# Excalibur-SLE/spmv

Measured on AMD Instinct MI355X. Metric: fp64 CG iters/sec (SpMV effective GB/s vs HBM roofline), higher is better.
Workload: dtype f64

## Files before the change

spmv_amd/csrc/hip/common.h:

```cpp
#pragma once

#include <mutex>
#include <vector>

#include <hip/hip_runtime.h>

#include <cstdint>
#include <cstdlib>

#include "spmv_hip.h"

struct spmv_hip_ctx {
  int device = 0;
  int num_cus = 0;
  hipStream_t stream = nullptr;
  int dot_blocks = 0;
  int64_t blas1_nt_min_elems = (int64_t)1 << 24;
  int64_t lx_min_nnz = (int64_t)1 << 20;
  int64_t lx_max_x_bytes = INT64_MAX;
  int lx_dma = 1;
  int lx_codes = 1;
  int lx_narrow_values = 1;
  int release_csr = 0;
  int64_t xw_min_nnz = (int64_t)1 << 20;
  int64_t xw_min_x_bytes = (int64_t)128 << 20;
  int xw_probe = 1;
  int csr_in_place = 0;
  int64_t lat_min_nnz = (int64_t)1 << 20;
  int bake_general = 1;
  int wdia_half = 1;
  int const_diagonals = 1;
  int const_tile = 4;
  int64_t sj_min_nnz = (int64_t)1 << 20;
  int sj_max_chunks = 432;
  int sj_wpb = 0;
  int sj_unit = 0;
  int sj_sigma = 1;
  int sym_sj_long_permille = 50;
  int sym_sj_long_rows = 1;
  int put_timeout_ms = 60000;
  std::vector<const int32_t*> watched;
  std::mutex watched_mutex;
  int poisson_skew_ppm = 0;
  int poisson_stencil = 7;
};

enum PeerWait : int32_t {
  kWaitNone = 0,
  kWaitPutFree = 1,
  kWaitPutData = 2,
  kWaitReduceSlot = 3
};
constexpr int kPeerErrLabels = 12;
constexpr int kPeerErrWords = kPeerErrLabels + 16;

// ... 95 lines not shown
```

spmv_amd/csrc/hip/csr_plan.h:

```cpp
#pragma once

#include "common.h"

#include <chrono>
#include <cstdio>

constexpr int kRows = kBlock;

typedef double f64x2 __attribute__((ext_vector_type(2)));
typedef float f32x4 __attribute__((ext_vector_type(4)));
typedef int i32x2 __attribute__((ext_vector_type(2)));
typedef int i32x4 __attribute__((ext_vector_type(4)));

template <typename T>
struct VecOf;
template <>
struct VecOf<double> {
  static constexpr int V = 2;
  using val_t = f64x2;
  using col_t = i32x2;
};
template <>
struct VecOf<float> {
  static constexpr int V = 4;
// ... 70 lines not shown
  }
}
__device__ __forceinline__ int order_slot_decode(const RowBlockOrder& ord,
                                                 int raw)
{
  const int rb = __builtin_amdgcn_readfirstlane(raw);
  return rb < ord.num_row_blocks ? rb : -1;
}
#endif

constexpr int kLxMaxWin = 16;
constexpr int kLxRec = 36;
constexpr int kLxCap = 1344;
constexpr int kLxGap = 16;
constexpr int kLxwPiece = 128;
constexpr int kLxwMaxPieces = 16;
constexpr int kLxwPieces0 = 4;
constexpr int kLxwNpMask = 0xff;
constexpr int kLxwOwnShift = 8;
constexpr int kLxwOwnMask = 0xfffff;
constexpr int kLxwCodedBit = 30;
constexpr int kLxwDict0 = kLxwPieces0 + kLxwMaxPieces;
constexpr int kLxwDictSize = 16;
constexpr int kLxwRec = 28;
__host__ __device__ constexpr int64_t lx_code_bytes(int64_t nnz)
{
  return (((nnz + 1) >> 1) + 16 + 15) & ~(int64_t)15;
}
__host__ __device__ constexpr int64_t lx32_len(int64_t nnz)
{
  return (nnz + 3) & ~(int64_t)3;
}
constexpr int kLxwAlign = 4;
constexpr int kXwMaxWin = 8;
constexpr int kXwFirst0 = kLxwPieces0 + kLxwMaxPieces;
constexpr int kXwDelta0 = kXwFirst0 + kXwMaxWin;
constexpr int kXwRec = 36;

constexpr int kLatMaxOff = 8;
constexpr int kLatRec = 12;
constexpr int kWdiaMaxOff = 32;

struct PlanTrace {
  bool on;
  std::chrono::steady_clock::time_point t0;
  const char* who;
  explicit PlanTrace(const char* w)
      : on(getenv("SPMV_PLAN_TRACE") != nullptr), t0(std::chrono::steady_clock::now()),
        who(w)
  {
  }
  void mark(const char* what) const
  {
    if (!on)
      return;
    (void)hipDeviceSynchronize();
    fprintf(stderr, "%s %-14s %9.3f ms\n", who, what,
            std::chrono::duration<double, std::milli>(std::chrono::steady_clock::now()
                                                      - t0)
                .count());
  }
};

template <typename T>
static inline bool aligned16(const T* p)
{
// ... 139 lines not shown
  int mv_form = 0;
  int mv_native = 1;
  int32_t* row_list = nullptr;
  int rowlist_exact = 0;
  int32_t num_listed = 0;
  int nt_store = 0;
  int plan_us = 0;
  int plan_mem_us = 0;
  int values_changed_us = 0;
  const int32_t* rowptr0 = nullptr;
  const int32_t* colind0 = nullptr;
  int released = 0;
  int no_new_forms = 0;
  bool structure_baked() const
  {
    return row_list || lx_lidx || lat_tab || slat_mask || t_ptr || lxw_rec
           || xw_rec || wdia_val || sj_lenperm;
  }
  uint16_t* lx_lidx = nullptr;
  int32_t* lx_tab = nullptr;
  int lx = 0;
  int lx_chunks = 2;
  int lx_staged = 0;
  int lx_blocks = 0;
  int32_t* lxw_rec = nullptr;
  int lxw = 0;
  int lxw_max_cnt = 0;
  int lxw_max_pieces = 0;
  int lxw_blocks_per_cu = 0;
  uint8_t* lx_code = nullptr;
  int lx4 = 0;
  int lx4_blocks = 0;
  int lx4_lut = 1;
  float* lx_val32 = nullptr;
  const void* lx32_values0 = nullptr;
  int lx_v32 = 0;
  int32_t* xw_rec = nullptr;
  int xw = 0;
  int xw_staged = 0;
  int xw_max_cnt = 0, xw_max_pieces = 0;
  struct XwProbe* xw_probe = nullptr;
  int32_t* lat_tab = nullptr;
  uint8_t* lat_mask = nullptr;
  int lat = 0;
  int lat_blocks = 0;
  int lat_blocks_per_cu = 4;
  int lat_xcd_group = 0;
  int lat_chain = 1;

  int lattice_d1 = 0, lattice_d2 = 0;

  int32_t* zw_table = nullptr;
  int zw_slots = 0;
  int zw_grid = 0;
  int zw_segments = 0;
  int64_t zw_d2 = 0;
  int zwalk = 0;

  RowBlockOrder row_block_order(int nrb) const
  {
    RowBlockOrder o;
    o.table = nullptr;
    o.num_slots = 0;
    o.xcd_group = xcd_group;
    o.num_row_blocks = nrb;
    o.nt_store = nt_store;
// ... 54 lines not shown
int spmv_zwalk_table_device(const spmv_hip_csr_plan* pl, int64_t rows,
                            int64_t d2, int grid, int segments, bool force,
                            int32_t** table, int* slots, int* segs);
int spmv_walk_grid(const spmv_hip_csr_plan* pl);
int spmv_slat_build(spmv_hip_csr_plan* pl, const int32_t* rowptr,
                    const int32_t* colind);
void spmv_slat_free(spmv_hip_csr_plan* pl);
int spmv_slat_grid(const spmv_hip_csr_plan* pl);
int spmv_slat_run_f64(const spmv_hip_csr_plan* pl, hipStream_t st,
                      const int32_t* rowptr, const double* values,
                      const double* diagonal, double alpha, const double* in,
                      double beta, double* out, DotOut dot);
int spmv_slat_run_f32(const spmv_hip_csr_plan* pl, hipStream_t st,
                      const int32_t* rowptr, const float* values,
                      const float* diagonal, float alpha, const float* in,
                      float beta, float* out);
void spmv_sdia_free(spmv_hip_csr_plan* pl);
int spmv_sdia_tile_build(spmv_hip_csr_plan* pl, int R, int segments, bool force);
int spmv_sdia_bake_f64(spmv_hip_csr_plan* pl, const double* values,
                       const double* diagonal, hipStream_t st);
int spmv_sdia_bake_f32(spmv_hip_csr_plan* pl, const float* values,
                       const float* diagonal, hipStream_t st);
int spmv_sdia_grid(const spmv_hip_csr_plan* pl);
int spmv_sdia_bake_f32f64(spmv_hip_csr_plan* pl, const float* values32,
                          hipStream_t st);
int spmv_sdia_run_f32f64(const spmv_hip_csr_plan* pl, hipStream_t st,
                         double alpha, const double* in, double beta,
                         double* out, DotOut dot);
int spmv_sdia_run_f64(const spmv_hip_csr_plan* pl, hipStream_t st, double alpha,
                      const double* in, double beta, double* out, DotOut dot);
int spmv_sdia_run_f32(const spmv_hip_csr_plan* pl, hipStream_t st, float alpha,
                      const float* in, float beta, float* out);
int spmv_lxw_grid(const spmv_hip_csr_plan* pl, int elem_bytes);
int spmv_lxw_run_f64(const spmv_hip_csr_plan* pl, hipStream_t st,
                     const int32_t* rowptr, const int32_t* colind,
                     const double* values, double alpha, const double* in,
                     double beta, double* out, DotOut dot);
int spmv_lxw_run_f32f64(const spmv_hip_csr_plan* pl, hipStream_t st,
                        const int32_t* rowptr, const int32_t* colind,
                        const float* values, double alpha, const double* in,
                        double beta, double* out, DotOut dot);
int spmv_xw_grid(const spmv_hip_csr_plan* pl, int elem_bytes);
int spmv_xw_run_f64(const spmv_hip_csr_plan* pl, hipStream_t st,
                    const int32_t* rowptr, const int32_t* colind,
                    const double* values, double alpha, const double* in,
                    double beta, double* out, DotOut dot);
int spmv_xw_run_f32(const spmv_hip_csr_plan* pl, hipStream_t st,
                    const int32_t* rowptr, const int32_t* colind,
                    const float* values, float alpha, const float* in,
                    float beta, float* out);
int spmv_lxw_run_f32(const spmv_hip_csr_plan* pl, hipStream_t st,
                     const int32_t* rowptr, const int32_t* colind,
                     const float* values, float alpha, const float* in,
                     float beta, float* out);
void spmv_wdia_free(spmv_hip_csr_plan* pl);
int spmv_wdia_walk_build(spmv_hip_csr_plan* pl, int segments, bool force);
int spmv_wdia_box_build(spmv_hip_csr_plan* pl, int R, int segments, bool force);
int spmv_wdia_hbox_build(spmv_hip_csr_plan* pl, int on);
int spmv_wdia_bake_f64(spmv_hip_csr_plan* pl, const double* values,
                       hipStream_t st);
int spmv_wdia_bake_f32(spmv_hip_csr_plan* pl, const float* values,
                       hipStream_t st);
int spmv_wdia_run_f64(const spmv_hip_csr_plan* pl, hipStream_t st, double alpha,
                      const double* in, double beta, double* out, DotOut dot);
int spmv_wdia_run_f32(const spmv_hip_csr_plan* pl, hipStream_t st, float alpha,
                      const float* in, float beta, float* out);
// ... 46 lines not shown
```

spmv_amd/csrc/hip/runtime.hip:

```cpp
#include "common.h"

#include <cstdio>
#include <cstring>
#include <new>

bool spmv_ctx_watch(spmv_hip_ctx* ctx, const int32_t* word, bool add)
{
  std::lock_guard<std::mutex> lock(ctx->watched_mutex);
  auto& ws = ctx->watched;
  if (add) {
    try {
      ws.push_back(word);
    } catch (...) {
      return false;
    }
    return true;
  }
  for (size_t i = 0; i < ws.size(); ++i)
    if (ws[i] == word) {
      ws[i] = ws.back();
      ws.pop_back();
      break;
    }
  return true;
// ... 111 lines not shown
  SPMV_REQUIRE(ctx && device_id);
  *device_id = ctx->device;
  return SPMV_HIP_OK;
}

int spmv_hip_num_cus(const spmv_hip_ctx* ctx, int* num_cus)
{
  SPMV_REQUIRE(ctx && num_cus);
  *num_cus = ctx->num_cus;
  return SPMV_HIP_OK;
}

int spmv_hip_ctx_get_option(const spmv_hip_ctx* ctx, const char* key, int64_t* value)
{
  SPMV_REQUIRE(ctx && key && value);
  if (!strcmp(key, "release_csr"))
    *value = ctx->release_csr;
  else if (!strcmp(key, "put_timeout_ms"))
    *value = ctx->put_timeout_ms;
  else if (!strcmp(key, "xw_min_nnz"))
    *value = ctx->xw_min_nnz;
  else if (!strcmp(key, "xw_min_x_bytes"))
    *value = ctx->xw_min_x_bytes;
  else if (!strcmp(key, "xw_probe"))
    *value = ctx->xw_probe;
  else if (!strcmp(key, "csr_in_place"))
    *value = ctx->csr_in_place;
  else if (!strcmp(key, "lx_min_nnz"))
    *value = ctx->lx_min_nnz;
  else if (!strcmp(key, "lat_min_nnz"))
    *value = ctx->lat_min_nnz;
  else if (!strcmp(key, "lx_narrow_values"))
    *value = ctx->lx_narrow_values;
  else if (!strcmp(key, "sj_min_nnz"))
    *value = ctx->sj_min_nnz;
  else
    return SPMV_HIP_EINVAL;
  return SPMV_HIP_OK;
}

int spmv_hip_ctx_set_option(spmv_hip_ctx* ctx, const char* key, int64_t value)
{
  SPMV_REQUIRE(ctx && key);
  if (!strcmp(key, "blas1_nt_min_elems")) {
    SPMV_REQUIRE(value >= 0);
    ctx->blas1_nt_min_elems = value;
    return SPMV_HIP_OK;
  }
  if (!strcmp(key, "lx_max_x_bytes")) {
    SPMV_REQUIRE(value >= 0);
    ctx->lx_max_x_bytes = value;
    return SPMV_HIP_OK;
  }
  if (!strcmp(key, "lx_min_nnz")) {
    SPMV_REQUIRE(value >= 0);
    ctx->lx_min_nnz = value;
    return SPMV_HIP_OK;
  }
  if (!strcmp(key, "release_csr")) {
    SPMV_REQUIRE(value == 0 || value == 1);
    ctx->release_csr = (int)value;
    return SPMV_HIP_OK;
  }
  if (!strcmp(key, "xw_min_x_bytes")) {
    SPMV_REQUIRE(value >= 0);
    ctx->xw_min_x_bytes = value;
// ... 7 lines not shown
  if (!strcmp(key, "xw_probe")) {
    SPMV_REQUIRE(value == 0 || value == 1);
    ctx->xw_probe = (int)value;
    return SPMV_HIP_OK;
  }
  if (!strcmp(key, "csr_in_place")) {
    SPMV_REQUIRE(value == 0 || value == 1);
    ctx->csr_in_place = (int)value;
    return SPMV_HIP_OK;
  }
  if (!strcmp(key, "lat_min_nnz")) {
    SPMV_REQUIRE(value >= 0);
    ctx->lat_min_nnz = value;
    return SPMV_HIP_OK;
  }
  if (!strcmp(key, "poisson_skew_ppm")) {
    SPMV_REQUIRE(value >= 0 && value < 1000000);
    ctx->poisson_skew_ppm = (int)value;
    return SPMV_HIP_OK;
  }
  if (!strcmp(key, "lx_dma")) {
    SPMV_REQUIRE(value == 0 || value == 1);
    ctx->lx_dma = (int)value;
    return SPMV_HIP_OK;
  }
  if (!strcmp(key, "lx_codes")) {
    SPMV_REQUIRE(value == 0 || value == 1);
    ctx->lx_codes = (int)value;
    return SPMV_HIP_OK;
  }
  if (!strcmp(key, "lx_narrow_values")) {
    SPMV_REQUIRE(value == 0 || value == 1);
    ctx->lx_narrow_values = (int)value;
    return SPMV_HIP_OK;
  }
  if (!strcmp(key, "poisson_stencil")) {
    SPMV_REQUIRE(value == 7 || value == 27);
    ctx->poisson_stencil = (int)value;
    return SPMV_HIP_OK;
  }
  if (!strcmp(key, "const_diagonals")) {
    SPMV_REQUIRE(value == 0 || value == 1);
    ctx->const_diagonals = (int)value;
    return SPMV_HIP_OK;
  }
  if (!strcmp(key, "const_tile")) {
    SPMV_REQUIRE(value == 1 || value == 2 || value == 4);
    ctx->const_tile = (int)value;
    return SPMV_HIP_OK;
  }
  if (!strcmp(key, "wdia_half")) {
    SPMV_REQUIRE(value == 0 || value == 1);
    ctx->wdia_half = (int)value;
    return SPMV_HIP_OK;
  }
  if (!strcmp(key, "sj_min_nnz")) {
    SPMV_REQUIRE(value >= 0);
    ctx->sj_min_nnz = value;
    return SPMV_HIP_OK;
  }
  if (!strcmp(key, "sj_max_chunks")) {
    SPMV_REQUIRE(value >= 8 && value <= 432);
    ctx->sj_max_chunks = (int)value;
    return SPMV_HIP_OK;
  }
  if (!strcmp(key, "sj_wpb")) {
// ... 254 lines not shown
```

spmv_amd/csrc/hip/spmv_csr_forms.hip:

```cpp
#include "csr_plan.h"

#include <hipcub/hipcub.hpp>

#include <algorithm>
#include <chrono>
#include <cstring>
#include <new>
#include <utility>
#include <vector>

#include "plan_scratch.h"

namespace
{

template <int ITEMS>
__global__ __launch_bounds__(kBlock) void lx_build_kernel(
    int32_t num_rows, int32_t num_cols, const int32_t* __restrict__ rowptr,
    const int32_t* __restrict__ colind, uint16_t* __restrict__ lidx,
    int32_t* __restrict__ tab, int num_row_blocks, int end_bit, int align,
    int pad, int cap, int32_t* __restrict__ wrec, int32_t* __restrict__ stat,
    int xw)
{
  using Sort = hipcub::BlockRadixSort<int32_t, kBlock, ITEMS, int32_t>;
// ... 108 lines not shown
      int np = 0;
      for (int k = 0; k < total_windows; ++k)
        for (int c = s_ws[k]; c < s_we[k]; c += kLxwPiece)
          wr[kLxwPieces0 + np++] = c;
      wr[0] = total_windows;
      int own = -1;
      for (int k = 0; k < total_windows; ++k)
        if (s_ws[k] <= r0 && r0 + nr <= s_we[k])
          own = s_wo[k] + (r0 - s_ws[k]);
      wr[3] = np | ((own + 1) << kLxwOwnShift);
      if (cnt > *(volatile int*)&stat[0])
        atomicMax(&stat[0], cnt);
      if (np > *(volatile int*)&stat[1])
        atomicMax(&stat[1], np);
      if (xw)
        atomicAdd(&stat[2], 1);
    }
  }
}

constexpr int kLx4Dmin = -kRows;
constexpr int kLx4Words = (kLxwMaxPieces * kLxwPiece + kRows + 31) / 32;
__global__ __launch_bounds__(kBlock) void lx4_encode_kernel(
    int32_t num_rows, const int32_t* __restrict__ rowptr,
    const uint16_t* __restrict__ lidx, int32_t* __restrict__ wrec,
    uint32_t* __restrict__ code, int num_row_blocks, int32_t* __restrict__ stat)
{
  constexpr int CAP = kBlock * 16;
  __shared__ uint32_t s_bits[kLx4Words];
  __shared__ int32_t s_rank[kLx4Words + 1];
  __shared__ int32_t s_dict[kLxwDictSize];
  __shared__ uint32_t s_pack[CAP / 8 + 2];
  const int t = threadIdx.x;
  int coded = 0;
  for (int rb = blockIdx.x; rb < num_row_blocks; rb += gridDim.x) {
    int32_t* wr = wrec + (int64_t)rb * kLxwRec;
    const int32_t a = wr[1], cnt = wr[2];
    const int nwin = wr[0];
    __syncthreads();
    if (nwin < 0 || cnt <= 0 || cnt > CAP)
      continue;
    const int32_t a0 = a & ~7;
    const int nwords = (int)(((int64_t)a + cnt + 7 - a0) >> 3);
    for (int w = t; w < kLx4Words; w += kBlock)
      s_bits[w] = 0;
    for (int w = t; w < nwords; w += kBlock)
      s_pack[w] = 0;
    if (t < kLxwDictSize)
      s_dict[t] = 0;
    __syncthreads();
    const int32_t r = rb * kRows + t;
    int32_t lo = 0, hi = 0;
    if (r < num_rows) {
      lo = rowptr[r];
      hi = rowptr[r + 1];
    }
    for (int32_t j = lo; j < hi; ++j) {
      const int b = (int)lidx[j] - t - kLx4Dmin;
      atomicOr(&s_bits[b >> 5], 1u << (b & 31));
    }
    __syncthreads();
    if (t == 0) {
      int n = 0;
      for (int w = 0; w < kLx4Words; ++w) {
        s_rank[w] = n;
        n += __popc(s_bits[w]);
      }
// ... 2 lines not shown
    __syncthreads();
    if (s_rank[kLx4Words] > kLxwDictSize)
      continue;
    for (int w = t; w < kLx4Words; w += kBlock) {
      uint32_t m = s_bits[w];
      int k = s_rank[w];
      while (m) {
        const int b = __ffs(m) - 1;
        m &= m - 1;
        s_dict[k++] = w * 32 + b + kLx4Dmin;
      }
    }
    for (int32_t j = lo; j < hi; ++j) {
      const int b = (int)lidx[j] - t - kLx4Dmin;
      const uint32_t c
          = (uint32_t)(s_rank[b >> 5] + __popc(s_bits[b >> 5] & ((1u << (b & 31)) - 1u)));
      const int q = j - a0;
      atomicOr(&s_pack[q >> 3], c << ((q & 7) * 4));
    }
    __syncthreads();
    for (int w = t; w < nwords; w += kBlock) {
      const bool whole = (w > 0 || a0 == a) && (int64_t)a0 + 8 * (w + 1) <= (int64_t)a + cnt;
      uint32_t* dst = code + ((int64_t)a0 >> 3) + w;
      if (whole)
        *dst = s_pack[w];
      else if (s_pack[w])
        atomicOr(dst, s_pack[w]);
    }
    if (t < kLxwDictSize / 2)
      wr[kLxwDict0 + t] = (s_dict[2 * t] & 0xffff) | (s_dict[2 * t + 1] << 16);
    if (t == 0) {
      wr[3] |= 1 << kLxwCodedBit;
      ++coded;
    }
  }
  if (t == 0 && coded)
    atomicAdd(&stat[0], coded);
}

struct NonEmptyRow {
  const int32_t* rowptr;
  __device__ bool operator()(int i) const { return rowptr[i + 1] > rowptr[i]; }
};

}

void xw_probe_free(spmv_hip_csr_plan* pl)
{
  if (!pl->xw_probe)
    return;
  for (auto& e : pl->xw_probe->ev)
    for (hipEvent_t& h : e)
      if (h) {
        (void)hipEventDestroy(h);
        h = nullptr;
      }
  delete pl->xw_probe;
  pl->xw_probe = nullptr;
}

void xw_probe_drop_events(XwProbe* pb)
{
  for (auto& e : pb->ev)
    for (hipEvent_t& h : e)
      if (h) {
        (void)hipEventDestroy(h);
        h = nullptr;
      }
}

// ... 39 lines not shown
  const size_t cap = (size_t)(pl->nnz < n ? pl->nnz : n);
  PlanScratch<int32_t> d_count;
  PlanScratch<void> tmp;
  SPMV_CHECK_HIP(spmv_plan_malloc(&pl->row_list, sizeof(int32_t) * (cap ? cap : 1)));
  hipError_t e = d_count.alloc(1);
  hipcub::CountingInputIterator<int32_t> first(0);
  NonEmptyRow pred{rowptr};
  if (e == hipSuccess)
    e = plan_cub(tmp, [&](void* t, size_t& tb) {
      return hipcub::DeviceSelect::If(t, tb, first, pl->row_list, d_count.get(), n,
                                      pred, st);
    });
  int32_t count = 0;
  if (e == hipSuccess)
    e = plan_fetch(&count, d_count.get(), 1, st);
  tmp.reset();
  d_count.reset();
  if (e != hipSuccess) {
    plan_drop(pl->row_list);
    return static_cast<int>(e);
  }
  pl->num_listed = count;
  return SPMV_HIP_OK;
}

void spmv_free_lx(spmv_hip_csr_plan* pl)
{
  plan_drop(pl->lx_lidx);
  plan_drop(pl->lx_tab);
  plan_drop(pl->lxw_rec);
  plan_drop(pl->lx_code);
  pl->lx = pl->lx_staged = pl->lx_blocks = 0;
  pl->lxw = pl->lxw_max_cnt = pl->lxw_max_pieces = 0;
  pl->lx4 = pl->lx4_blocks = 0;
  spmv_lx32_free(pl);
}

static int build_lx_codes(spmv_hip_csr_plan* pl, const int32_t* rowptr, int nrb,
                          hipStream_t st)
{
  const size_t bytes = (size_t)lx_code_bytes(pl->nnz);
  PlanScratch<int32_t> d_stat;
  hipError_t e = spmv_plan_malloc(&pl->lx_code, bytes);
  if (e == hipSuccess)
    e = d_stat.alloc(1);
  if (e == hipSuccess)
    e = hipMemsetAsync(pl->lx_code, 0, bytes, st);
  if (e == hipSuccess)
    e = hipMemsetAsync(d_stat.get(), 0, sizeof(int32_t), st);
  int32_t coded = 0;
  if (e == hipSuccess) {
    int grid = pl->ctx->num_cus * 8;
    grid = grid > nrb ? nrb : grid;
    hipLaunchKernelGGL(lx4_encode_kernel, dim3(grid), dim3(kBlock), 0, st,
                       pl->num_rows, rowptr, pl->lx_lidx, pl->lxw_rec,
                       reinterpret_cast<uint32_t*>(pl->lx_code), nrb, d_stat.get());
    e = hipGetLastError();
  }
  if (e == hipSuccess)
    e = plan_fetch(&coded, d_stat.get(), 1, st);
  d_stat.reset();
  if (e != hipSuccess || coded == 0) {
    (void)hipGetLastError();
    plan_drop(pl->lx_code);
    pl->lx4 = pl->lx4_blocks = 0;
    return e == hipSuccess || e == hipErrorOutOfMemory ? SPMV_HIP_OK
                                                       : static_cast<int>(e);
  }
  pl->lx4_blocks = coded;
  pl->lx4 = 1;
  return SPMV_HIP_OK;
}

namespace
{

__device__ __forceinline__ bool lx32_exact(double v)
{
  const double a = fabs(v);
  if (!(a == 0.0 || (a >= 0x1p-126 && a <= 0x1.fffffep+127)))
    return false;
  return __double_as_longlong((double)(float)v) == __double_as_longlong(v);
}

__global__ __launch_bounds__(kBlock) void lx32_check_kernel(
    int64_t nnz, const double* __restrict__ values, int32_t* __restrict__ flag)
{
  const f64x2* v2 = reinterpret_cast<const f64x2*>(values);
  const int64_t pairs = nnz >> 1;
  bool bad = false;
  for (int64_t i = (int64_t)blockIdx.x * kBlock + threadIdx.x; i < pairs;
       i += (int64_t)gridDim.x * kBlock) {
    const f64x2 v = v2[i];
    bad |= !lx32_exact(v.x) || !lx32_exact(v.y);
  }
  if ((nnz & 1) && blockIdx.x == 0 && threadIdx.x == 0)
    bad |= !lx32_exact(values[nnz - 1]);
  if (bad)
    atomicOr(flag, 1);
}

__global__ __launch_bounds__(kBlock) void lx32_convert_kernel(
// ... 496 lines not shown
```

spmv_amd/csrc/hip/spmv_csr_plan.hip:

```cpp
#include "csr_plan.h"

#include <hipcub/hipcub.hpp>

#include <algorithm>
#include <chrono>
#include <cstring>
#include <new>
#include <utility>
#include <vector>

#include "plan_scratch.h"

thread_local int64_t spmv_plan_mem_ns = 0;

namespace
{
struct MemClock {
  spmv_hip_csr_plan* pl;
  int64_t t0;
  explicit MemClock(spmv_hip_csr_plan* p = nullptr) : pl(p), t0(spmv_plan_mem_ns) {}
  ~MemClock()
  {
    if (pl)
      pl->plan_mem_us += (int)((spmv_plan_mem_ns - t0) / 1000);
// ... 55 lines not shown
               : 0;
  if (pl->sdia32_val || pl->wdia32_val || pl->sj_val32)
    return 0;
  if (pl->sdia && pl->sdia_val && pl->sdia_general && pl->sdia_values0)
    return 3;
  if (pl->wdia && pl->wdia_val && pl->wdia_values0)
    return 3;
  if (pl->sj && pl->sj_val && pl->sj_values0 && pl->sj_nlong == 0 && pl->num_cols >= 2)
    return 3;
  return 0;
}

extern "C" {

int spmv_hip_csr_plan_create(spmv_hip_ctx* ctx, int32_t num_rows,
                             int32_t num_cols, int64_t num_non_zeros,
                             const int32_t* rowptr, const int32_t* colind,
                             int symmetric, int algo, spmv_hip_csr_plan** plan)
{
  SPMV_REQUIRE(ctx && plan && num_rows >= 0 && num_cols >= 0
               && num_non_zeros >= 0);
  SPMV_REQUIRE(num_non_zeros == 0 || (rowptr && colind));
  if (num_non_zeros > 0) {
    SPMV_SET_DEVICE(ctx);
    SPMV_CHECK_HIP(hipStreamSynchronize(spmv_stream(ctx, nullptr)));
  }
  const auto t_begin = std::chrono::steady_clock::now();
  if (num_non_zeros > INT32_MAX)
    return SPMV_HIP_ERANGE;
  spmv_hip_csr_plan* pl = new (std::nothrow) spmv_hip_csr_plan;
  if (!pl)
    return SPMV_HIP_ENOMEM;
  pl->ctx = ctx;
  MemClock mem_clock(pl);
  pl->num_rows = num_rows;
  pl->num_cols = num_cols;
  pl->nnz = num_non_zeros;
  pl->symmetric = symmetric != 0;
  pl->rowptr0 = rowptr;
  pl->colind0 = colind;
  const double avg = num_rows > 0 ? (double)num_non_zeros / num_rows : 0.0;
  if (algo == SPMV_HIP_ALGO_AUTO) {
    if (!symmetric && num_non_zeros > 0 && num_non_zeros * 4 < num_rows)
      algo = SPMV_HIP_ALGO_ROWLIST;
    else
      algo = (avg <= 64.0 || num_non_zeros >= ctx->sj_min_nnz)
                 ? SPMV_HIP_ALGO_ROWBLOCK
                 : SPMV_HIP_ALGO_VECTOR;
  }
  if (algo < SPMV_HIP_ALGO_ROWBLOCK || algo > SPMV_HIP_ALGO_ROWLIST
      || (algo == SPMV_HIP_ALGO_ROWLIST && (symmetric || num_non_zeros == 0))) {
    mem_clock.pl = nullptr;
    delete pl;
    return SPMV_HIP_EINVAL;
  }
  pl->algo = algo;
  if (algo == SPMV_HIP_ALGO_ROWLIST) {
    int rc = spmv_build_row_list(pl, rowptr);
    if (rc != SPMV_HIP_OK) {
      mem_clock.pl = nullptr;
      delete pl;
      return rc;
    }
  }
  int lpr = 4;
  while (lpr < 64 && lpr < avg / 2)
// ... 343 lines not shown
  } else if (!strcmp(key, "xcd_group")) {
    SPMV_REQUIRE(value >= 0 && value <= 4096);
    plan->xcd_group = value;
  } else if (!strcmp(key, "sym_window")) {
    SPMV_REQUIRE(value >= 0 && value <= 4096 && value % 256 == 0);
    plan->sym_window = value;
  } else if (!strcmp(key, "sym_rows")) {
    SPMV_REQUIRE(value == 512 || value == 1024 || value == 2048);
    plan->sym_rows = value;
  } else if (!strcmp(key, "blocks_per_cu")) {
    SPMV_REQUIRE(value >= 1 && value <= kBlocksPerCU);
    plan->blocks_per_cu = value;
    if (plan->zw_table && !plan->lat_tab && !plan->symmetric
        && !plan->sdia_val)
      return spmv_zwalk_order_build(plan, plan->zw_d2, spmv_walk_grid(plan), 0,
                                    true);
  } else if (!strcmp(key, "lx")) {
    SPMV_REQUIRE(value == 0 || plan->lx_lidx);
    plan->lx = value != 0;
  } else if (!strcmp(key, "lxw")) {
    SPMV_REQUIRE(value == 0 || plan->lxw_rec);
    plan->lxw = value != 0;
    if (plan->zw_table && plan->lx_lidx && !plan->lat_tab)
      return spmv_zwalk_order_build(plan, plan->zw_d2, spmv_walk_grid(plan), 0,
                                    true);
  } else if (!strcmp(key, "lx4")) {
    SPMV_REQUIRE(value == 0 || value == 1);
    SPMV_REQUIRE(value == 0 || plan->lx_code);
    plan->lx4 = value;
  } else if (!strcmp(key, "lx_v32")) {
    SPMV_REQUIRE(value == 0 || value == 1);
    SPMV_REQUIRE(value == 0 || plan->lx_val32);
    plan->lx_v32 = value;
  } else if (!strcmp(key, "lx4_lut")) {
    SPMV_REQUIRE(value == 1 || value == 2);
    plan->lx4_lut = value;
  } else if (!strcmp(key, "xw")) {
    SPMV_REQUIRE(value == 0 || plan->xw_rec);
    plan->xw = value != 0;
    if (plan->xw_probe && value) {
      plan->xw_probe->decided = 1;
      plan->xw_probe->use_xw = 1;
    }
    if (plan->zw_table && plan->xw_rec && !plan->lat_tab && !plan->lx_lidx)
      return spmv_zwalk_order_build(plan, plan->zw_d2, spmv_walk_grid(plan), 0,
                                    true);
  } else if (!strcmp(key, "xw_probe")) {
    SPMV_REQUIRE((value == 0 || value == 1) && plan->xw_rec);
    if (!plan->xw_probe)
      plan->xw_probe = new (std::nothrow) XwProbe;
    SPMV_REQUIRE(plan->xw_probe);
    xw_probe_drop_events(plan->xw_probe);
    *plan->xw_probe = XwProbe();
    plan->xw_probe->decided = value ? 0 : 1;
  } else if (!strcmp(key, "lxw_blocks_per_cu")) {
    SPMV_REQUIRE(value >= 0 && value <= kBlocksPerCU);
    plan->lxw_blocks_per_cu = value;
    if (plan->zw_table && !plan->lat_tab
        && ((plan->lxw_rec && plan->lxw) || (plan->xw_rec && plan->xw)))
      return spmv_zwalk_order_build(plan, plan->zw_d2, spmv_walk_grid(plan), 0,
                                    true);
  } else if (!strcmp(key, "lx_chunks")) {
    SPMV_REQUIRE(value == 1 || value == 2);
    plan->lx_chunks = value;
  } else if (!strcmp(key, "nt_store")) {
    plan->nt_store = value != 0;
// ... 333 lines not shown
    *value = plan->sdia_chain;
  else if (!strcmp(key, "sdia_nt"))
    *value = plan->sdia_nt;
  else if (!strcmp(key, "zwalk"))
    *value = plan->zwalk && plan->zw_table ? 1 : 0;
  else if (!strcmp(key, "zwalk_segments"))
    *value = plan->zw_table ? plan->zw_segments : 0;
  else if (!strcmp(key, "zwalk_grid"))
    *value = plan->zw_table ? plan->zw_grid : 0;
  else if (!strcmp(key, "lattice_d1"))
    *value = plan->lattice_d1;
  else if (!strcmp(key, "lattice_d2"))
    *value = plan->lattice_d2;
  else if (!strcmp(key, "lat"))
    *value = plan->lat;
  else if (!strcmp(key, "lat_chain"))
    *value = plan->lat_chain;
  else if (!strcmp(key, "lat_blocks"))
    *value = plan->lat_blocks;
  else if (!strcmp(key, "lx"))
    *value = plan->lx;
  else if (!strcmp(key, "lxw"))
    *value = plan->lxw && plan->lxw_rec ? 1 : 0;
  else if (!strcmp(key, "lx4"))
    *value = plan->lx4 && plan->lx_code ? 1 : 0;
  else if (!strcmp(key, "lx4_blocks"))
    *value = plan->lx_code ? plan->lx4_blocks : 0;
  else if (!strcmp(key, "lx4_all"))
    *value = plan->lx_code && plan->lx4_blocks == plan->lx_staged ? 1 : 0;
  else if (!strcmp(key, "lx4_lut"))
    *value = plan->lx4_lut;
  else if (!strcmp(key, "lx_v32"))
    *value = plan->lx_v32 && plan->lx_val32 ? 1 : 0;
  else if (!strcmp(key, "lxw_grid"))
    *value = plan->lxw_rec ? spmv_lxw_grid(plan, 8) : 0;
  else if (!strcmp(key, "lx_staged"))
    *value = plan->lx_staged;
  else if (!strcmp(key, "lx_blocks"))
    *value = plan->lx_blocks;
  else if (!strcmp(key, "blocks_per_cu"))
    *value = plan->blocks_per_cu;
  else if (!strcmp(key, "nontemporal"))
    *value = plan->nontemporal;
  else
    return spmv_tr_get(plan, key, value);
  return SPMV_HIP_OK;
}

}
```

spmv_amd/csrc/hip/spmv_lxw.hip:

```cpp
#include "csr_plan.h"
#include "lat_dma.h"

#include <new>
#include <type_traits>

namespace
{

struct LxwBlock {
  int rb;
  int nwin;
  int32_t a;
  int32_t cnt;
  int np;
  int own;
  int coded;
};

template <int REC>
__device__ __forceinline__ int32_t lxw_fetch(int rb,
                                             const int32_t* __restrict__ rec)
{
  int32_t w = 0;
  if (rb >= 0) {
// ... 315 lines not shown
      const T c = alpha * sum;
      T y = c;
      if (beta != T(0))
        y = c + beta * g.y0;
      y_late = y;
      r_late = r;
      if constexpr (DOT) {
        if (!own_staged)
          x_own = in[r];
        dot_acc += (double)x_own * (double)c;
      }
    }
    slot ^= 1;
    cur = nxt;
    cur_ws = nxt_ws;
    cur_dc = nxt_dc;
    nxt_rb = nn_rb;
    nxt_w = nn_w;
    nn_raw = nnn_raw;
    it += stride;
  };
  while (it < num_slots) {
    step(gA, gB);
    if (it >= num_slots)
      break;
    step(gB, gA);
  }
  if (r_late >= 0)
    out[r_late] = y_late;
  if constexpr (DOT)
    spmv_dot_epilogue(dot, dot_acc, s_red);
}

struct LxwGeom {
  int vcap, lcap, xcap;
  size_t lds;
  int per_cu;
};

LxwGeom lxw_geom(const spmv_hip_csr_plan* pl, int elem_bytes, int idx_bytes)
{
  LxwGeom g;
  const bool xw = idx_bytes == 4;
  const int V = 16 / elem_bytes;
  const int max_cnt = xw ? pl->xw_max_cnt : pl->lxw_max_cnt;
  int64_t vb = ((int64_t)(max_cnt + V) * elem_bytes + 1023) & ~1023ll;
  vb = vb < 1024 ? 1024 : (vb > 32768 ? 32768 : vb);
  g.vcap = (int)(vb / elem_bytes);
  int64_t lb = ((int64_t)(g.vcap + 8) * idx_bytes + 1023) & ~1023ll;
  g.lcap = (int)(lb / idx_bytes);
  int np = xw ? pl->xw_max_pieces : pl->lxw_max_pieces;
  np = np < 1 ? 1 : np;
  g.xcap = np * kLxwPiece;
  g.lds = 2 * (size_t)vb + 2 * (size_t)lb + 2 * (size_t)g.xcap * elem_bytes;
  int per = (int)((160 * 1024 - 1024) / (g.lds + 64));
  per = per < 1 ? 1 : (per > kBlocksPerCU ? kBlocksPerCU : per);
  if (pl->lxw_blocks_per_cu > 0 && pl->lxw_blocks_per_cu < per)
    per = pl->lxw_blocks_per_cu;
  g.per_cu = per;
  return g;
}

int lxw_grid(const spmv_hip_csr_plan* pl, int elem_bytes, int idx_bytes)
{
  const LxwGeom g = lxw_geom(pl, elem_bytes, idx_bytes);
  const int nrb = (pl->num_rows + kRows - 1) / kRows;
  int grid = pl->ctx->num_cus * g.per_cu;
  if (grid > pl->ctx->dot_blocks)
    grid = pl->ctx->dot_blocks;
  if (grid > nrb)
    grid = nrb;
  if (grid < 1)
    grid = 1;
  if (grid >= 8)
    grid -= grid % 8;
  return grid;
}

template <typename TV, typename T, bool DOT, bool XW, int C4>
int lxw_launch_c(const spmv_hip_csr_plan* pl, hipStream_t st,
                 const int32_t* rowptr, const int32_t* colind, const TV* values,
                 T alpha, const T* in, T beta, T* out, DotOut dot)
{
  const LxwGeom g = lxw_geom(pl, (int)sizeof(T), XW ? 4 : 2);
  const int vcap = g.vcap * (int)(sizeof(T) / sizeof(TV));
  const int nrb = (pl->num_rows + kRows - 1) / kRows;
  const int grid = lxw_grid(pl, (int)sizeof(T), XW ? 4 : 2);
  RowBlockOrder ord = pl->row_block_order(nrb);
  ord.xcd_group = pl->lat_xcd_group;
  if (pl->zwalk && pl->zw_table && pl->zw_grid == grid) {
    ord.table = pl->zw_table;
    ord.num_slots = pl->zw_slots;
  }
  auto kern
      = ord.table
            ? (pl->nontemporal ? csr_lxw_kernel<TV, T, DOT, true, true, XW, C4>
                               : csr_lxw_kernel<TV, T, DOT, false, true, XW, C4>)
            : (pl->nontemporal ? csr_lxw_kernel<TV, T, DOT, true, false, XW, C4>
                               : csr_lxw_kernel<TV, T, DOT, false, false, XW, C4>);
  if (g.lds > 48 * 1024)
    SPMV_CHECK_HIP(hipFuncSetAttribute(
        reinterpret_cast<const void*>(kern),
        hipFuncAttributeMaxDynamicSharedMemorySize, (int)g.lds));
  hipLaunchKernelGGL(kern, dim3(grid), dim3(kBlock), g.lds, st, pl->num_rows,
                     pl->num_cols, pl->nnz, rowptr, colind, values,
                     XW ? nullptr : pl->lx_lidx, C4 ? pl->lx_code : nullptr,
                     XW ? pl->xw_rec : pl->lxw_rec, alpha, in, beta, out, dot,
                     ord, vcap, g.lcap, g.xcap);
  SPMV_CHECK_LAUNCH();
  return SPMV_HIP_OK;
}

template <typename TV, typename T, bool DOT, bool XW>
int lxw_launch(const spmv_hip_csr_plan* pl, hipStream_t st,
               const int32_t* rowptr, const int32_t* colind, const TV* values,
               T alpha, const T* in, T beta, T* out, DotOut dot)
{
  if constexpr (!XW) {
    if (pl->lx4 && pl->lx_code)
      return pl->lx4_lut == 2
                 ? lxw_launch_c<TV, T, DOT, XW, 2>(pl, st, rowptr, colind, values,
                                                   alpha, in, beta, out, dot)
                 : lxw_launch_c<TV, T, DOT, XW, 1>(pl, st, rowptr, colind, values,
                                                   alpha, in, beta, out, dot);
  }
  return lxw_launch_c<TV, T, DOT, XW, 0>(pl, st, rowptr, colind, values, alpha,
                                         in, beta, out, dot);
}

}

int spmv_lxw_grid(const spmv_hip_csr_plan* pl, int elem_bytes)
{
  return lxw_grid(pl, elem_bytes, 2);
}

int spmv_xw_grid(const spmv_hip_csr_plan* pl, int elem_bytes)
{
  return lxw_grid(pl, elem_bytes, 4);
}

int spmv_lxw_run_f64(const spmv_hip_csr_plan* pl, hipStream_t st,
                     const int32_t* rowptr, const int32_t* colind,
                     const double* values, double alpha, const double* in,
                     double beta, double* out, DotOut dot)
{
  if (dot.partials)
    return lxw_launch<double, double, true, false>(pl, st, rowptr, colind, values,
                                                   alpha, in, beta, out, dot);
  return lxw_launch<double, double, false, false>(pl, st, rowptr, colind, values,
                                                  alpha, in, beta, out, dot);
}

int spmv_lxw_run_f32f64(const spmv_hip_csr_plan* pl, hipStream_t st,
                        const int32_t* rowptr, const int32_t* colind,
                        const float* values, double alpha, const double* in,
                        double beta, double* out, DotOut dot)
{
  if (dot.partials)
    return lxw_launch<float, double, true, false>(pl, st, rowptr, colind, values,
                                                  alpha, in, beta, out, dot);
  return lxw_launch<float, double, false, false>(pl, st, rowptr, colind, values,
                                                 alpha, in, beta, out, dot);
}

int spmv_lxw_run_f32(const spmv_hip_csr_plan* pl, hipStream_t st,
                     const int32_t* rowptr, const int32_t* colind,
                     const float* values, float alpha, const float* in,
                     float beta, float* out)
// ... 26 lines not shown
```

Before: 294.4.

## Add triple-buffered ring pipeline kernel for coded LXW SpMV with f32 values

Adds a new LXW SpMV kernel that keeps three LDS slots and issues the global-to-LDS loads for values, 4-bit codes and x pieces two row blocks ahead. Row pointers, y and records are loaded with inline-asm loads and partial vmcnt waits, so compute on the current block overlaps memory traffic for later ones. The plan-building pass now counts which blocks fit the ring, and the ring path is chosen only when every block fits, LDS occupancy is no worse and there are enough steps per block. This trades more LDS per block and fragile hand-placed waitcnt asm for hiding load latency.

```diff
diff --git a/spmv_amd/csrc/hip/common.h b/spmv_amd/csrc/hip/common.h
--- a/spmv_amd/csrc/hip/common.h
+++ b/spmv_amd/csrc/hip/common.h
@@ -21,6 +21,7 @@
   int lx_dma = 1;
   int lx_codes = 1;
   int lx_narrow_values = 1;
+  int lx_ring = 1;
   int release_csr = 0;
   int64_t xw_min_nnz = (int64_t)1 << 20;
   int64_t xw_min_x_bytes = (int64_t)128 << 20;
diff --git a/spmv_amd/csrc/hip/csr_plan.h b/spmv_amd/csrc/hip/csr_plan.h
--- a/spmv_amd/csrc/hip/csr_plan.h
+++ b/spmv_amd/csrc/hip/csr_plan.h
@@ -126,6 +126,18 @@
   return (nnz + 3) & ~(int64_t)3;
 }
 constexpr int kLxwAlign = 4;
+constexpr int kLxwRingValRounds = 2;
+constexpr int kLxwRingVcap = kLxwRingValRounds * 1024;
+constexpr int kLxwRingCodeMax = 4096;
+__host__ __device__ constexpr int lx_ring_code_bytes(int cnt)
+{
+  return (cnt + 31 + 7) / 8 * 4 + 8;
+}
+__host__ __device__ constexpr bool lx_ring_fits(int cnt)
+{
+  return cnt > 0 && cnt + 3 <= kLxwRingVcap
+         && lx_ring_code_bytes(cnt) <= kLxwRingCodeMax;
+}
 constexpr int kXwMaxWin = 8;
 constexpr int kXwFirst0 = kLxwPieces0 + kLxwMaxPieces;
 constexpr int kXwDelta0 = kXwFirst0 + kXwMaxWin;
@@ -331,6 +343,8 @@
   int lx4 = 0;
   int lx4_blocks = 0;
   int lx4_lut = 1;
+  int lx_ring_blocks = 0;
+  int lx_ring = 1;
   float* lx_val32 = nullptr;
   const void* lx32_values0 = nullptr;
   int lx_v32 = 0;
@@ -451,6 +465,7 @@
 int spmv_sdia_run_f32(const spmv_hip_csr_plan* pl, hipStream_t st, float alpha,
                       const float* in, float beta, float* out);
 int spmv_lxw_grid(const spmv_hip_csr_plan* pl, int elem_bytes);
+bool spmv_lxw_ring_ok(const spmv_hip_csr_plan* pl, bool forced);
 int spmv_lxw_run_f64(const spmv_hip_csr_plan* pl, hipStream_t st,
                      const int32_t* rowptr, const int32_t* colind,
                      const double* values, double alpha, const double* in,
diff --git a/spmv_amd/csrc/hip/runtime.hip b/spmv_amd/csrc/hip/runtime.hip
--- a/spmv_amd/csrc/hip/runtime.hip
+++ b/spmv_amd/csrc/hip/runtime.hip
@@ -167,6 +167,8 @@
     *value = ctx->lat_min_nnz;
   else if (!strcmp(key, "lx_narrow_values"))
     *value = ctx->lx_narrow_values;
+  else if (!strcmp(key, "lx_ring"))
+    *value = ctx->lx_ring;
   else if (!strcmp(key, "sj_min_nnz"))
     *value = ctx->sj_min_nnz;
   else
@@ -240,6 +242,11 @@
   if (!strcmp(key, "lx_narrow_values")) {
     SPMV_REQUIRE(value == 0 || value == 1);
     ctx->lx_narrow_values = (int)value;
+    return SPMV_HIP_OK;
+  }
+  if (!strcmp(key, "lx_ring")) {
+    SPMV_REQUIRE(value >= 0 && value <= 2);
+    ctx->lx_ring = (int)value;
     return SPMV_HIP_OK;
   }
   if (!strcmp(key, "poisson_stencil")) {
diff --git a/spmv_amd/csrc/hip/spmv_csr_forms.hip b/spmv_amd/csrc/hip/spmv_csr_forms.hip
--- a/spmv_amd/csrc/hip/spmv_csr_forms.hip
+++ b/spmv_amd/csrc/hip/spmv_csr_forms.hip
@@ -164,7 +164,7 @@
   __shared__ int32_t s_dict[kLxwDictSize];
   __shared__ uint32_t s_pack[CAP / 8 + 2];
   const int t = threadIdx.x;
-  int coded = 0;
+  int coded = 0, ring = 0;
   for (int rb = blockIdx.x; rb < num_row_blocks; rb += gridDim.x) {
     int32_t* wr = wrec + (int64_t)rb * kLxwRec;
     const int32_t a = wr[1], cnt = wr[2];
@@ -233,10 +233,13 @@
     if (t == 0) {
       wr[3] |= 1 << kLxwCodedBit;
       ++coded;
+      ring += lx_ring_fits(cnt) ? 1 : 0;
     }
   }
   if (t == 0 && coded)
     atomicAdd(&stat[0], coded);
+  if (t == 0 && ring)
+    atomicAdd(&stat[1], ring);
 }
 
 struct NonEmptyRow {
@@ -342,7 +345,7 @@
   plan_drop(pl->lx_code);
   pl->lx = pl->lx_staged = pl->lx_blocks = 0;
   pl->lxw = pl->lxw_max_cnt = pl->lxw_max_pieces = 0;
-  pl->lx4 = pl->lx4_blocks = 0;
+  pl->lx4 = pl->lx4_blocks = pl->lx_ring_blocks = 0;
   spmv_lx32_free(pl);
 }
 
@@ -353,12 +356,12 @@
   PlanScratch<int32_t> d_stat;
   hipError_t e = spmv_plan_malloc(&pl->lx_code, bytes);
   if (e == hipSuccess)
-    e = d_stat.alloc(1);
+    e = d_stat.alloc(2);
   if (e == hipSuccess)
     e = hipMemsetAsync(pl->lx_code, 0, bytes, st);
   if (e == hipSuccess)
-    e = hipMemsetAsync(d_stat.get(), 0, sizeof(int32_t), st);
-  int32_t coded = 0;
+    e = hipMemsetAsync(d_stat.get(), 0, 2 * sizeof(int32_t), st);
+  int32_t h_stat[2] = {0, 0};
   if (e == hipSuccess) {
     int grid = pl->ctx->num_cus * 8;
     grid = grid > nrb ? nrb : grid;
@@ -368,16 +371,18 @@
     e = hipGetLastError();
   }
   if (e == hipSuccess)
-    e = plan_fetch(&coded, d_stat.get(), 1, st);
+    e = plan_fetch(h_stat, d_stat.get(), 2, st);
   d_stat.reset();
+  const int32_t coded = h_stat[0];
   if (e != hipSuccess || coded == 0) {
     (void)hipGetLastError();
     plan_drop(pl->lx_code);
-    pl->lx4 = pl->lx4_blocks = 0;
+    pl->lx4 = pl->lx4_blocks = pl->lx_ring_blocks = 0;
     return e == hipSuccess || e == hipErrorOutOfMemory ? SPMV_HIP_OK
                                                        : static_cast<int>(e);
   }
   pl->lx4_blocks = coded;
+  pl->lx_ring_blocks = h_stat[1];
   pl->lx4 = 1;
   return SPMV_HIP_OK;
 }
diff --git a/spmv_amd/csrc/hip/spmv_csr_plan.hip b/spmv_amd/csrc/hip/spmv_csr_plan.hip
--- a/spmv_amd/csrc/hip/spmv_csr_plan.hip
+++ b/spmv_amd/csrc/hip/spmv_csr_plan.hip
@@ -111,6 +111,7 @@
   if (!pl)
     return SPMV_HIP_ENOMEM;
   pl->ctx = ctx;
+  pl->lx_ring = ctx->lx_ring;
   MemClock mem_clock(pl);
   pl->num_rows = num_rows;
   pl->num_cols = num_cols;
@@ -520,6 +521,10 @@
     SPMV_REQUIRE(value == 0 || value == 1);
     SPMV_REQUIRE(value == 0 || plan->lx_val32);
     plan->lx_v32 = value;
+  } else if (!strcmp(key, "lx_ring")) {
+    SPMV_REQUIRE(value == 0 || value == 1);
+    SPMV_REQUIRE(value == 0 || spmv_lxw_ring_ok(plan, true));
+    plan->lx_ring = value ? 2 : 0;
   } else if (!strcmp(key, "lx4_lut")) {
     SPMV_REQUIRE(value == 1 || value == 2);
     plan->lx4_lut = value;
@@ -919,6 +924,10 @@
     *value = plan->lx4_lut;
   else if (!strcmp(key, "lx_v32"))
     *value = plan->lx_v32 && plan->lx_val32 ? 1 : 0;
+  else if (!strcmp(key, "lx_ring"))
+    *value = spmv_lxw_ring_ok(plan, false) ? 1 : 0;
+  else if (!strcmp(key, "lx_ring_blocks"))
+    *value = plan->lx_code ? plan->lx_ring_blocks : 0;
   else if (!strcmp(key, "lxw_grid"))
     *value = plan->lxw_rec ? spmv_lxw_grid(plan, 8) : 0;
   else if (!strcmp(key, "lx_staged"))
diff --git a/spmv_amd/csrc/hip/spmv_lxw.hip b/spmv_amd/csrc/hip/spmv_lxw.hip
--- a/spmv_amd/csrc/hip/spmv_lxw.hip
+++ b/spmv_amd/csrc/hip/spmv_lxw.hip
@@ -371,6 +371,252 @@
     spmv_dot_epilogue(dot, dot_acc, s_red);
 }
 
+__device__ __forceinline__ int32_t ring_ld32(const int32_t* p)
+{
+  int32_t v;
+  asm volatile("global_load_dword %0, %1, off" : "=v"(v) : "v"(p) : "memory");
+  return v;
+}
+__device__ __forceinline__ double ring_ld64(const double* p)
+{
+  double v;
+  asm volatile("global_load_dwordx2 %0, %1, off" : "=v"(v) : "v"(p) : "memory");
+  return v;
+}
+__device__ __forceinline__ void ring_st64(double* p, double v)
+{
+  asm volatile("global_store_dwordx2 %0, %1, off" : : "v"(p), "v"(v) : "memory");
+}
+template <int N>
+__device__ __forceinline__ void ring_wait(int32_t& a, int32_t& b, double& c,
+                                          int32_t& d, int32_t& e)
+{
+  asm volatile("s_waitcnt vmcnt(%5)"
+               : "+v"(a), "+v"(b), "+v"(c), "+v"(d), "+v"(e)
+               : "n"(N)
+               : "memory");
+}
+
+template <bool DOT, bool NT, bool TAB, int VR, int PWR>
+__global__ __launch_bounds__(kBlock) void csr_lxw_ring_kernel(
+    int32_t num_rows, int32_t num_cols, int64_t nnz,
+    const int32_t* __restrict__ rowptr, const float* __restrict__ values,
+    const uint8_t* __restrict__ code, const int32_t* __restrict__ rec,
+    double alpha, const double* __restrict__ in, double beta,
+    double* __restrict__ out, DotOut dot, RowBlockOrder ord, int ccap, int xcap)
+{
+  using T = double;
+  constexpr int NW = kBlock / 64;
+  constexpr int VCAP = VR * NW * 256;
+  constexpr int DMA = VR + 1 + PWR;
+  extern __shared__ __attribute__((aligned(16))) unsigned char smem[];
+  float* const s_val = reinterpret_cast<float*>(smem);
+  unsigned char* const s_code = smem + 3 * (size_t)VCAP * sizeof(float);
+  T* const s_x = reinterpret_cast<T*>(s_code + 3 * (size_t)ccap);
+  __shared__ double s_red[NW];
+  __shared__ int32_t s_dict[3 * kLxwDictSize / 2];
+  const unsigned lds_val = (unsigned)(uintptr_t)(
+      (__attribute__((address_space(3))) void*)s_val);
+  const unsigned lds_code = lds_val + 3u * VCAP * (unsigned)sizeof(float);
+  const unsigned lds_x = lds_code + 3u * (unsigned)ccap;
+  const unsigned lds_dump = lds_x + 3u * (unsigned)xcap * (unsigned)sizeof(T);
+
+  const int t = threadIdx.x;
+  const int wave = __builtin_amdgcn_readfirstlane(t >> 6);
+  const int lane = t & 63;
+  const int stride = gridDim.x;
+  const int num_slots = order_slots(ord);
+  double dot_acc = 0.0;
+  const int32_t col_last = (num_cols - 2) & ~1;
+  const int64_t code_len = lx_code_bytes(nnz);
+  const int64_t val_len = lx32_len(nnz);
+  const int64_t vdump = lane * 4 < val_len - 4 ? lane * 4 : val_len - 4;
+  const int64_t cdump = lane * 16 < code_len - 16 ? lane * 16 : code_len - 16;
+  const int32_t xdump = lane * 2 < col_last ? lane * 2 : col_last;
+
+  auto issue = [&](const LxwBlock& b, int32_t w, int sl) {
+    const bool live = b.rb >= 0;
+    const int64_t a = b.a, e = (int64_t)b.a + b.cnt;
+    {
+      const int64_t base = a & ~(int64_t)3;
+      const int64_t jclamp = (e - 1) & ~(int64_t)3;
+      const int pieces = live ? (int)(((e - base) * 4 + 1023) >> 10) : 0;
+#pragma unroll
+      for (int r = 0; r < VR; ++r) {
+        const int q = wave + NW * r;
+        const bool real = q < pieces;
+        int64_t j = base + (int64_t)(q * 64 + lane) * 4;
+        j = j < jclamp ? j : jclamp;
+        j = real ? j : vdump;
+        glds16<NT>(values + j,
+                   real ? lds_val + (unsigned)(sl * VCAP * 4 + q * 1024)
+                        : lds_dump);
+      }
+    }
+    {
+      const int64_t base = (a >> 1) & ~(int64_t)15, end = (e + 1) >> 1;
+      const int64_t jclamp = (end - 1) & ~(int64_t)15;
+      const int pieces = live ? (int)((end - base + 1023) >> 10) : 0;
+      const bool real = wave < pieces;
+      int64_t j = base + (int64_t)(wave * 64 + lane) * 16;
+      j = j < jclamp ? j : jclamp;
+      j = real ? j : cdump;
+      glds16<NT>(code + j, real ? lds_code + (unsigned)(sl * ccap + wave * 1024)
+                                : lds_dump);
+    }
+    const int np = live ? b.np : 0;
+#pragma unroll
+    for (int k = 0; k < PWR; ++k) {
+      const int p = wave + NW * k;
+      const bool real = p < np;
+      const int32_t col = __builtin_amdgcn_readlane(w, kLxwPieces0 + p);
+      int32_t c = col + lane * 2;
+      c = c < col_last ? c : col_last;
+      c = real ? c : xdump;
+      glds16<false>(in + c,
+                    real ? lds_x + (unsigned)((sl * xcap + p * kLxwPiece) * 8)
+                         : lds_dump);
+    }
+  };
+  auto put_dict = [&](const LxwBlock& b, int32_t w, int sl) {
+    if (b.rb >= 0 && t >= kLxwDict0 && t < kLxwDict0 + kLxwDictSize / 2)
+      s_dict[sl * (kLxwDictSize / 2) + t - kLxwDict0] = w;
+  };
+  auto raw_of = [&](int i) {
+    if constexpr (TAB)
+      return ring_ld32(ord.table + (i < num_slots ? i : num_slots - 1));
+    else
+      return order_slot_raw_t<false>(ord, i, num_slots);
+  };
+  auto rb_of = [&](int i, int raw) {
+    return i < num_slots ? order_slot_decode(ord, raw) : -1;
+  };
+  auto fetch = [&](int rb) {
+    return ring_ld32(rec + (int64_t)(rb < 0 ? 0 : rb) * kLxwRec
+                     + (lane < kLxwRec ? lane : kLxwRec - 1));
+  };
+  auto loads = [&](int rb, int32_t& lo, int32_t& hi, double& y0) {
+    int32_t r = (rb < 0 ? 0 : rb) * kRows + t;
+    r = r < num_rows ? r : num_rows - 1;
+    lo = ring_ld32(rowptr + r);
+    hi = ring_ld32(rowptr + r + 1);
+    y0 = ring_ld64(out + (beta != 0.0 ? r : (t < num_rows ? t : num_rows - 1)));
+  };
+
+  int it = blockIdx.x;
+  int32_t raw0 = raw_of(it), raw1 = raw_of(it + stride);
+  int32_t raw2 = raw_of(it + 2 * stride), raw3 = raw_of(it + 3 * stride);
+  double dz = 0.0;
+  ring_wait<0>(raw0, raw1, dz, raw2, raw3);
+  const int rb0 = rb_of(it, raw0), rb1 = rb_of(it + stride, raw1);
+  int rb2 = rb_of(it + 2 * stride, raw2);
+  int32_t w0 = fetch(rb0), w1 = fetch(rb1), w2 = fetch(rb2);
+  int32_t iz = 0;
+  ring_wait<0>(w0, w1, dz, w2, iz);
+  LxwBlock cur = lxw_decode(rb0, w0);
+  LxwBlock nxt = lxw_decode(rb1, w1);
+  put_dict(cur, w0, 0);
+  put_dict(nxt, w1, 1);
+  issue(cur, w0, 0);
+  issue(nxt, w1, 1);
+  int32_t lo, hi;
+  double y0;
+  loads(cur.rb, lo, hi, y0);
+  ring_wait<0>(lo, hi, y0, iz, iz);
+  __syncthreads();
+  int s0 = 0, s2 = 2;
+  T y_late = T(0);
+  int32_t r_late = -1;
+
+  while (it < num_slots) {
+    if (r_late >= 0)
+      ring_st64(out + r_late, y_late);
+    r_late = -1;
+    int32_t nlo, nhi;
+    double ny0;
+    loads(nxt.rb, nlo, nhi, ny0);
+    const int rb3 = rb_of(it + 3 * stride, raw3);
+    int32_t w3 = fetch(rb3);
+    int32_t raw4 = raw_of(it + 4 * stride);
+    const LxwBlock blk2 = lxw_decode(rb2, w2);
+    put_dict(blk2, w2, s2);
+    issue(blk2, w2, s2);
+
+    const int32_t r = cur.rb * kRows + t;
+    if (cur.rb >= 0 && r < num_rows) {
+      T sum = 0;
+      T x_own = T(0);
+      int32_t j = lo;
+      const float* sv = s_val + (size_t)s0 * VCAP + (cur.a & 3) - cur.a;
+      const T* sx = s_x + (size_t)s0 * xcap;
+      if constexpr (DOT) {
+        if (cur.own >= 0)
+          x_own = sx[cur.own + t];
+      }
+      const uint32_t* sc
+          = reinterpret_cast<const uint32_t*>(s_code + (size_t)s0 * ccap);
+      const int32_t n0 = cur.a & ~31;
+      for (; j < hi; j += 8) {
+        const unsigned n = (unsigned)(j - n0);
+        const uint32_t c_lo = sc[n >> 3], c_hi = sc[(n >> 3) + 1];
+        const uint32_t bits = __builtin_amdgcn_alignbit(c_hi, c_lo, (n & 7) * 4);
+        unsigned l[8];
+        T v[8], xv[8];
+#pragma unroll
+        for (int k = 0; k < 8; ++k) {
+          const int32_t jj = j + k < hi ? j + k : hi - 1;
+          v[k] = (T)sv[jj];
+        }
+#pragma unroll
+        for (int k = 0; k < 8; ++k) {
+          const unsigned c = (bits >> (4 * k)) & 15u;
+          const int32_t d = reinterpret_cast<const int16_t*>(
+              s_dict + s0 * (kLxwDictSize / 2))[c];
+          l[k] = j + k < hi ? (unsigned)(t + d) : 0u;
+        }
+#pragma unroll
+        for (int k = 0; k < 8; ++k)
+          xv[k] = sx[l[k]];
+#pragma unroll
+        for (int k = 0; k < 8; ++k)
+          if (j + k < hi)
+            sum += v[k] * xv[k];
+      }
+      const T c = alpha * sum;
+      T y = c;
+      if (beta != T(0))
+        y = c + beta * y0;
+      y_late = y;
+      r_late = r;
+      if constexpr (DOT) {
+        if (cur.own < 0) {
+          x_own = ring_ld64(in + r);
+          asm volatile("s_waitcnt vmcnt(0)" : "+v"(x_own) : : "memory");
+        }
+        dot_acc += (double)x_own * (double)c;
+      }
+    }
+    ring_wait<DMA>(nlo, nhi, ny0, w3, raw4);
+    __syncthreads();
+    cur = nxt;
+    nxt = blk2;
+    lo = nlo;
+    hi = nhi;
+    y0 = ny0;
+    rb2 = rb3;
+    w2 = w3;
+    raw3 = raw4;
+    s2 = s0;
+    s0 = s0 == 2 ? 0 : s0 + 1;
+    it += stride;
+  }
+  ring_wait<0>(lo, hi, y0, w2, raw3);
+  if (r_late >= 0)
+    ring_st64(out + r_late, y_late);
+  if constexpr (DOT)
+    spmv_dot_epilogue(dot, dot_acc, s_red);
+}
+
 struct LxwGeom {
   int vcap, lcap, xcap;
   size_t lds;
@@ -416,6 +662,77 @@
   return grid;
 }
 
+struct LxwRingGeom {
+  int ccap, xcap;
+  size_t lds;
+  int per_cu;
+};
+
+LxwRingGeom lxw_ring_geom(const spmv_hip_csr_plan* pl)
+{
+  LxwRingGeom g;
+  const int max_cnt = pl->lxw_max_cnt < 1 ? 1 : pl->lxw_max_cnt;
+  g.ccap = (lx_ring_code_bytes(max_cnt) + 1023) & ~1023;
+  int np = pl->lxw_max_pieces;
+  np = np < 1 ? 1 : np;
+  g.xcap = np * kLxwPiece;
+  g.lds = 3 * ((size_t)kLxwRingVcap * sizeof(float) + (size_t)g.ccap
+               + (size_t)g.xcap * sizeof(double))
+          + 1024;
+  g.per_cu = (int)((160 * 1024 - 1024) / (g.lds + 256));
+  return g;
+}
+
+bool lxw_ring_ok(const spmv_hip_csr_plan* pl, bool forced)
+{
+  const int nrb = (pl->num_rows + kRows - 1) / kRows;
+  if (!(forced || pl->lx_ring) || pl->symmetric || !pl->lx || !pl->lxw
+      || !pl->lxw_rec || !pl->lx4 || !pl->lx_code || pl->lx4_lut != 1
+      || !pl->lx_v32 || !pl->lx_val32)
+    return false;
+  if (nrb < 1 || pl->lx_staged != nrb || pl->lx4_blocks != nrb
+      || pl->lx_ring_blocks != nrb || !lx_ring_fits(pl->lxw_max_cnt)
+      || pl->lxw_max_pieces > kLxwMaxPieces)
+    return false;
+  if (lxw_ring_geom(pl).per_cu < lxw_geom(pl, 8, 2).per_cu)
+    return false;
+  constexpr int kMinSteps = 128;
+  const int grid = lxw_grid(pl, 8, 2);
+  return forced || pl->lx_ring >= 2 || (nrb + grid - 1) / grid >= kMinSteps;
+}
+
+template <bool DOT>
+int lxw_ring_launch(const spmv_hip_csr_plan* pl, hipStream_t st,
+                    const int32_t* rowptr, const float* values, double alpha,
+                    const double* in, double beta, double* out, DotOut dot)
+{
+  constexpr int VR = kLxwRingValRounds, PWR = kLxwMaxPieces / (kBlock / 64);
+  const LxwRingGeom g = lxw_ring_geom(pl);
+  const int nrb = (pl->num_rows + kRows - 1) / kRows;
+  const int grid = lxw_grid(pl, 8, 2);
+  RowBlockOrder ord = pl->row_block_order(nrb);
+  ord.xcd_group = pl->lat_xcd_group;
+  if (pl->zwalk && pl->zw_table && pl->zw_grid == grid) {
+    ord.table = pl->zw_table;
+    ord.num_slots = pl->zw_slots;
+  }
+  auto kern
+      = ord.table
+            ? (pl->nontemporal ? csr_lxw_ring_kernel<DOT, true, true, VR, PWR>
+                               : csr_lxw_ring_kernel<DOT, false, true, VR, PWR>)
+            : (pl->nontemporal ? csr_lxw_ring_kernel<DOT, true, false, VR, PWR>
+                               : csr_lxw_ring_kernel<DOT, false, false, VR, PWR>);
+  if (g.lds > 48 * 1024)
+    SPMV_CHECK_HIP(hipFuncSetAttribute(
+        reinterpret_cast<const void*>(kern),
+        hipFuncAttributeMaxDynamicSharedMemorySize, (int)g.lds));
+  hipLaunchKernelGGL(kern, dim3(grid), dim3(kBlock), g.lds, st, pl->num_rows,
+                     pl->num_cols, pl->nnz, rowptr, values, pl->lx_code,
+                     pl->lxw_rec, alpha, in, beta, out, dot, ord, g.ccap, g.xcap);
+  SPMV_CHECK_LAUNCH();
+  return SPMV_HIP_OK;
+}
+
 template <typename TV, typename T, bool DOT, bool XW, int C4>
 int lxw_launch_c(const spmv_hip_csr_plan* pl, hipStream_t st,
                  const int32_t* rowptr, const int32_t* colind, const TV* values,
@@ -455,6 +772,12 @@
                const int32_t* rowptr, const int32_t* colind, const TV* values,
                T alpha, const T* in, T beta, T* out, DotOut dot)
 {
+  if constexpr (!XW && std::is_same<TV, float>::value
+                && std::is_same<T, double>::value) {
+    if (lxw_ring_ok(pl, false))
+      return lxw_ring_launch<DOT>(pl, st, rowptr, values, alpha, in, beta, out,
+                                  dot);
+  }
   if constexpr (!XW) {
     if (pl->lx4 && pl->lx_code)
       return pl->lx4_lut == 2
@@ -474,6 +797,11 @@
   return lxw_grid(pl, elem_bytes, 2);
 }
 
+bool spmv_lxw_ring_ok(const spmv_hip_csr_plan* pl, bool forced)
+{
+  return lxw_ring_ok(pl, forced);
+}
+
 int spmv_xw_grid(const spmv_hip_csr_plan* pl, int elem_bytes)
 {
   return lxw_grid(pl, elem_bytes, 4);
```

Result: faster. 326.0, median of 6 (+10.7%).
